# Aedelon/MASt3R-SLAM

Measured on AMD Instinct MI355X. Metric: keyframe-pairs/sec (512x512 two-view infer+match+GN), higher is better.
Workload: dtype fp16

## Files before the change

mast3r-slam_amd/csrc/gemm.hip:

```cpp
#include <atomic>
#include "gemm_common.h"
#include <cmath>
#include <stdlib.h>

using namespace m3gemm;

namespace {

constexpr int BM = 128, BN = 128;
constexpr int kThreads = 256;

#ifndef M3_GEMM64_STAGES
#define M3_GEMM64_STAGES 2
#endif
constexpr int k_gemm_stages(int T) { return T == 64 ? M3_GEMM64_STAGES : 2; }

template <int MODE , int EPI, int T, int DT, bool SLICED = false>
__global__ void __launch_bounds__(kThreads)
k_gemm(const GemmArgs gin) {
    constexpr int BM = T, BN = T;
    constexpr int NT = T / 32;
    constexpr int kStageBytes = (BM + BN) * BK * 2;
    constexpr int STAGES = k_gemm_stages(T);
    static_assert(4 * (NT == 4 ? 9216 : 4608) + BM * 8 + kRopeTableRows * 128 <= STAGES * kStageBytes, "row table + RoPE table behind the scratch");
// ... 330 lines not shown
    store_tile<EPI, DT>(g, f32x4{a.x, a.y, a.z, a.w}, m, n);
}

template <int MODE>
int run_split(const GemmArgs &a, int S, int epi, void *ws, hipStream_t st) {
    if (MODE == 1 && (epi == EPI_BF16 || epi == EPI_BF16_RELU || epi == EPI_BF16_ADD)) {
        const long tiles = (long)m3_cdiv(a.M, BM) * m3_cdiv(a.N, BN) * (a.groups > 1 ? a.groups : 1);
        static const bool sliced_ok = [] { const char *e = getenv("M3_CONV_SLICED"); return !(e && atoi(e) == 0); }();
        if (sliced_ok && tiles >= m3_device_cu_count()) {
            GemmArgs q = a;
            q.slices = S; q.splits = 1;
            return launch<MODE>(q, epi, st);
        }
    }
    GemmArgs p = a;
    p.C = ws; p.ldc = a.N; p.bias = nullptr; p.bias2 = nullptr; p.R = nullptr; p.splits = S;
    p.c_gstride = (long long)S * a.M * a.N;
    const int rc = launch<MODE>(p, EPI_F32, st);
    if (rc != M3_OK) return rc;
    const dim3 grid((unsigned)m3_cdiv((long)a.M * (a.N / 4), 256L), a.groups > 1 ? a.groups : 1);
#define M3_F(E) case E:                                                                                        \
        if (a.dt == DT_F16) hipLaunchKernelGGL((k_splitk_finish<E, DT_F16>), grid, dim3(256), 0, st, a, (const float *)ws, S); \
        else hipLaunchKernelGGL((k_splitk_finish<E, DT_BF16>), grid, dim3(256), 0, st, a, (const float *)ws, S);      \
        break
    switch (epi) {
        M3_F(EPI_BF16); M3_F(EPI_BF16_GELU); M3_F(EPI_F32); M3_F(EPI_F32_ACCUM); M3_F(EPI_BF16_RELU); M3_F(EPI_BF16_ADD);
        default: return M3_ERR_INVALID_ARG;
    }
#undef M3_F
    M3_CHECK_LAUNCH("m3_gemm/splitk_finish");
    return M3_OK;
}

}

int m3_launch_gemm256_dense(const GemmArgs &a, int epi, int bn, hipStream_t st);
int m3_launch_gemm256_conv(const GemmArgs &a, int epi, hipStream_t st);

static int launch_dense(const GemmArgs &a, int epi, hipStream_t st) {
    const int tile = pick_tile(a.M, a.N, a.groups > 1 ? 2 : 1);
    if (tile >= 192) return m3_launch_gemm256_dense(a, epi, tile, st);
    if (tile == 64) return launch<0, 64>(a, epi, st);
    return launch<0>(a, epi, st);
}

extern "C" {

int m3_gemm_set_tile(int tile) { return g_forced_tile.exchange(tile, std::memory_order_relaxed); }

int m3_gemm_pick_tile(int M, int N, int groups) {
    if (M <= 0 || N <= 0) return 0;
    return pick_tile(M, N, groups > 1 ? groups : 1);
}

static bool dt_ok(int dtype) { return dtype == DT_BF16 || dtype == DT_F16; }

static int ln_top_width(int C) {
    if (C % 192 == 0 && C / 192 <= 4) return 192;
    if (C % 256 == 0 && C / 256 <= 4) return 256;
    return 0;
}
static int ln_store_width(int M, int N, int groups) {
    const int tile = pick_tile(M, N, groups), top = ln_top_width(N);
    if (top == 0) return 0;
    if (tile == top) return top;
    if (top == 256 && tile == 128) return 128;
    return 64;
}
int m3_ln_slot_count(int M, int N, int groups) {
    if (M <= 0 || N <= 0) return 0;
    const int w = ln_store_width(M, N, groups > 1 ? 2 : 1);
    return w ? N / w : 0;
}

int m3_gemm_ex(const m3_gemm_desc *d, void *stream) {
    M3_REQUIRE(d && d->A && d->W && (d->C || d->c_lo) && d->M > 0 && d->N > 0 && d->K > 0);
    const int epi = d->epilogue, groups = d->groups > 1 ? 2 : 1;
    const bool rope = epi == EPI_BF16_ROPE;
    M3_REQUIRE(dt_ok(d->dtype) || (rope && d->dtype == 2));
    M3_REQUIRE(d->K % BK == 0 && d->N % 4 == 0 && d->ldc >= d->N && d->ldc % 4 == 0);
    M3_REQUIRE(!((epi == EPI_F32_ACCUM || epi == EPI_BF16_ADD) && !d->R));
    M3_REQUIRE(epi >= EPI_BF16 && epi <= EPI_BF16_ROPE);
    if (d->c_lo)
        M3_REQUIRE((epi == EPI_F32 || epi == EPI_F32_ACCUM) && d->dtype == DT_F16 && d->c16 && !d->C && d->N % 8 == 0 && d->ldc % 8 == 0 &&
                   d->M % 2 == 0 && (reinterpret_cast<size_t>(d->c_lo) & 15) == 0 && (reinterpret_cast<size_t>(d->c16) & 15) == 0 &&
                   (epi == EPI_F32 || (d->r_lo && (reinterpret_cast<size_t>(d->R) & 15) == 0 && (reinterpret_cast<size_t>(d->r_lo) & 15) == 0)));
    if (groups == 2) M3_REQUIRE(d->W1 && (d->bias == nullptr) == (d->bias1 == nullptr));
    if (rope)
        M3_REQUIRE(d->rope_pos && d->tokens_per_image > 0 && d->rope_base > 1.0f && d->N % 64 == 0 && d->rope_cols % 64 == 0 &&
                   d->rope_cols <= d->N && d->q_cols >= 0 && d->q_cols <= d->rope_cols && d->q_cols % 64 == 0);
    const bool f32out = epi == EPI_F32 || epi == EPI_F32_ACCUM;
    if (d->c16 || d->stats_out) {
        M3_REQUIRE(f32out && (d->N % 64 == 0 || !d->stats_out) && d->M % 2 == 0 && d->ldc % 8 == 0 && (reinterpret_cast<size_t>(d->C) & 15) == 0 &&
                   (!d->R || (reinterpret_cast<size_t>(d->R) & 15) == 0) &&
                   (!d->c16 || (reinterpret_cast<size_t>(d->c16) & 15) == 0) &&
                   (!d->stats_out || (reinterpret_cast<size_t>(d->stats_out) & 15) == 0));
        if (groups == 2) M3_REQUIRE(d->c_gstride % 8 == 0 && d->stats_gstride % 4 == 0);
        if (d->stats_out) M3_REQUIRE(d->stats_slots > 0 && d->stats_slots == m3_ln_slot_count(d->M, d->N, groups));
    }
    if (d->ln_stats) {
        const int top = ln_top_width(d->K);
        M3_REQUIRE(top != 0 && (d->ln_slots == d->K / 64 || (top == 256 && d->ln_slots == d->K / 128) || d->ln_slots == d->K / top));
        M3_REQUIRE(!f32out && epi != EPI_BF16_ADD && d->ln_colsum &&
                   d->ln_eps > 0.0f && d->M % 2 == 0 && (reinterpret_cast<size_t>(d->ln_stats) & 15) == 0 &&
                   (reinterpret_cast<size_t>(d->ln_colsum) & 15) == 0 && (reinterpret_cast<size_t>(d->C) & 15) == 0 &&
                   d->ldc % 8 == 0 && d->N % 8 == 0);
        if (groups == 2) M3_REQUIRE(d->ln_colsum1 && (reinterpret_cast<size_t>(d->ln_colsum1) & 15) == 0 && d->ln_gstride % 4 == 0);
    }
    GemmArgs a{};
    a.A = (const bf16_t *)d->A; a.W = (const bf16_t *)d->W; a.W2 = (const bf16_t *)d->W1; a.bias = d->bias; a.bias2 = d->bias1;
    a.C = d->C; a.R = d->R; a.M = d->M; a.N = d->N; a.K = d->K; a.ldc = d->ldc;
    a.dt = d->dtype == 2 ? DT_F16 : d->dtype; a.v_bf16 = d->dtype == 2;
    a.a_gstride = d->a_gstride; a.c_gstride = d->c_gstride; a.groups = groups == 2 ? 2 : 0;
    if (rope) {
        a.rope_pos = d->rope_pos; a.rope_log2_base = log2f(d->rope_base); a.tokens_per_image = d->tokens_per_image;
        a.rope_cols = d->rope_cols; a.q_cols = d->q_cols; a.q_scale = d->q_scale;
        a.rope_pmax = (d->rope_max_pos > 0 && d->rope_max_pos <= kRopeTableRows) ? d->rope_max_pos : 0;
    }
    a.C16 = d->c16; a.stats_out = d->stats_out; a.stats_gstride = d->stats_gstride;
    a.R_lo = d->r_lo; a.C_lo = d->c_lo;
    a.ln_stats = d->ln_stats; a.ln_colsum = d->ln_colsum; a.ln_colsum2 = d->ln_colsum1; a.ln_slots = d->ln_slots;
    a.ln_eps = d->ln_eps; a.ln_gstride = d->ln_gstride;
    if (d->ln_stats) {
        const int top = ln_top_width(d->K);
        a.ln_tops = d->K / top;
        a.ln_gsz = d->ln_slots / a.ln_tops;
    }
    a.stats_w = d->stats_out ? ln_store_width(d->M, d->N, groups) : 0;
    return launch_dense(a, epi, (hipStream_t)stream);
}

int64_t m3_conv3x3_splitk_bytes(int B, int H, int Wd, int Cin, int Cout, int stride) {
    if (B <= 0 || H <= 0 || Wd <= 0 || Cin <= 0 || Cout <= 0 || (stride != 1 && stride != 2)) return 0;
    const int OH = (H + 2 - 3) / stride + 1, OW = (Wd + 2 - 3) / stride + 1;
    const int S = pick_splits(OH * OW, Cout, 9 * Cin);
    return S > 1 ? (int64_t)S * B * OH * OW * Cout * 4 : 0;
}

int m3_conv3x3_grouped2_dt(const void *X, const void *W0, const void *W1, const float *bias0, const float *bias1,
                           void *Y, const void *R, const void *zero16, int B, int H, int Wd, int Cin, int Cout,
                           int stride, int epilogue, void *splitk_ws, int64_t splitk_ws_bytes, int dtype, void *stream) {
    const int relu_in = (epilogue & 0x100) ? 1 : 0;
    epilogue &= 0xff;
    M3_REQUIRE(X && W0 && Y && zero16 && B > 0 && H > 0 && Wd > 0 && Cin > 0 && Cout > 0 && dt_ok(dtype));
    M3_REQUIRE(Cin % BK == 0 && Cout % 4 == 0 && (stride == 1 || stride == 2) && epilogue != EPI_BF16_ROPE);
    M3_REQUIRE(!((epilogue == EPI_F32_ACCUM || epilogue == EPI_BF16_ADD) && !R));
    M3_REQUIRE(!W1 || (bias0 == nullptr) == (bias1 == nullptr));
    GemmArgs a{};
    a.relu_a = relu_in;
    a.A = (const bf16_t *)X; a.W = (const bf16_t *)W0; a.bias = bias0; a.C = Y; a.R = R;
    a.zero16 = (const bf16_t *)zero16;
    a.H = H; a.Wd = Wd; a.Cin = Cin; a.stride = stride;
    a.OH = (H + 2 - 3) / stride + 1; a.OW = (Wd + 2 - 3) / stride + 1;
    a.M = B * a.OH * a.OW; a.N = Cout; a.K = 9 * Cin; a.ldc = Cout; a.dt = dtype;
    if (W1) {
        a.W2 = (const bf16_t *)W1; a.bias2 = bias1;
        a.groups = 2; a.a_gstride = (long long)B * H * Wd * Cin; a.c_gstride = (long long)a.M * Cout;
    }
    const int S = pick_splits(a.OH * a.OW, Cout, a.K);
    if (S > 1) {
        M3_REQUIRE(splitk_ws && (reinterpret_cast<size_t>(splitk_ws) & 15) == 0 &&
                   splitk_ws_bytes >= (W1 ? 2 : 1) * (int64_t)S * a.M * a.N * 4);
        return run_split<1>(a, S, epilogue, splitk_ws, (hipStream_t)stream);
    }
    if (use_256(a.M, a.N, W1 ? 2 : 1)) return m3_launch_gemm256_conv(a, epilogue, (hipStream_t)stream);
    return launch<1>(a, epilogue, (hipStream_t)stream);
}

int m3_conv3x3_relu_head4_dt(const void *X, const void *W, const float *bias, const void *W4, const float *b4,
                             float *pts, float *conf, const void *zero16, int B, int H, int Wd, int Cin, int dtype,
                             void *stream) {
    M3_REQUIRE(X && W && W4 && b4 && pts && conf && zero16 && B > 0 && H > 0 && Wd > 0 && Cin > 0 && Cin % BK == 0);
    M3_REQUIRE(dt_ok(dtype));
    M3_REQUIRE((int64_t)B * H * Wd < (1ll << 31));
    GemmArgs a{};
    a.A = (const bf16_t *)X; a.W = (const bf16_t *)W; a.bias = bias; a.C = pts; a.C2 = conf;
    a.W2 = (const bf16_t *)W4; a.bias2 = b4;
    a.zero16 = (const bf16_t *)zero16;
    a.H = H; a.Wd = Wd; a.Cin = Cin; a.stride = 1; a.OH = H; a.OW = Wd;
// ... 6 lines not shown
```

mast3r-slam_amd/csrc/gemm256.hip:

```cpp
#include "gemm_common.h"

using namespace m3gemm;

namespace {

constexpr int BM = 256;
constexpr int kThreads = 512;

template <int MODE , int EPI, int BN, int DT>
__global__ void __launch_bounds__(kThreads, 2)
k_gemm256(const GemmArgs gin) {
    constexpr int WN = BN == 256 ? 4 : 2, WM = 8 / WN;
    constexpr int NI = BM / WM / 16, NJ = BN / WN / 16;
    constexpr int WISS = BN / 64;
    constexpr int kStageBytes = (BM + BN) * BK * 2;
    static_assert(8 * (64 * (32 * NJ + 16)) + kRopeTableRows * 128 <= 2 * kStageBytes, "RoPE table behind the epilogue scratch");
    const GemmArgs g = select_group<EPI>(gin, blockIdx.y);
    extern __shared__ __attribute__((aligned(16))) unsigned char lds[];
    const int tid = threadIdx.x, lane = tid & 63, wave = tid >> 6;
    const int group = wave >> 2;
    const int wr = wave / WN, wc = wave % WN;

    const int tiles_n = (g.N + BN - 1) / BN, tiles_m = (g.M + BM - 1) / BM;
    const int bid = xcd_remap(blockIdx.x, tiles_m * tiles_n);
    constexpr int GM = 8;
    const int band = bid / (GM * tiles_n), first_m = band * GM;
    const int gsz = tiles_m - first_m < GM ? tiles_m - first_m : GM;
    const int in_band = bid - band * GM * tiles_n;
    const int tm = first_m + in_band % gsz, tn = in_band / gsz;
    const int m0 = tm * BM, n0 = tn * BN;

    const int srow = tid >> 3, sch = (tid & 7) ^ ((srow >> 1) & 7);
    const bf16_t *a_src[4];
    const bf16_t *w_src[WISS];
    int a_oy[4], a_ox[4];
    const bf16_t *a_img[4];
#pragma unroll
    for (int i = 0; i < WISS; ++i) {
        int n = n0 + i * 64 + srow;
        n = n < g.N ? n : g.N - 1;
        w_src[i] = g.W + (size_t)n * g.K + sch * 8;
    }
#pragma unroll
    for (int i = 0; i < 4; ++i) {
        int m = m0 + i * 64 + srow;
        m = m < g.M ? m : g.M - 1;
        if (MODE == 0) {
            a_src[i] = g.A + (size_t)m * g.K + sch * 8;
        } else {
            const int pix = g.OH * g.OW;
            const int b = m / pix, rem = m - b * pix;
            a_oy[i] = (rem / g.OW) * g.stride - 1;
            a_ox[i] = (rem % g.OW) * g.stride - 1;
            a_img[i] = g.A + (size_t)b * g.H * g.Wd * g.Cin + sch * 8;
        }
    }
    const int nk = g.K / BK;

    auto stage_a = [&](int kt, int buf) {
        unsigned char *base = lds + buf * kStageBytes;
        int ky = 0, kx = 0, c0 = 0;
        if (MODE == 1) {
            const int q = kt / 9, tap = kt - q * 9;
            c0 = q * BK;
            ky = tap / 3; kx = tap - ky * 3;
        }
#pragma unroll
        for (int i = 0; i < 4; ++i) {
            const void *src;
            if (MODE == 0) {
                src = a_src[i] + (size_t)kt * BK;
            } else {
                const int iy = a_oy[i] + ky, ix = a_ox[i] + kx;
                const bool in = (iy >= 0) && (iy < g.H) && (ix >= 0) && (ix < g.Wd);
                src = in ? (const void *)(a_img[i] + ((size_t)iy * g.Wd + ix) * g.Cin + c0) : (const void *)g.zero16;
            }
            glds16(src, base + i * 8192 + wave * 1024);
        }
    };
    auto stage_w = [&](int kt, int buf) {
        unsigned char *base = lds + buf * kStageBytes;
        const size_t koff = MODE == 1 ? conv_k_offset(kt, g.Cin) : (size_t)kt * BK;
#pragma unroll
        for (int i = 0; i < WISS; ++i)
            glds16(w_src[i] + koff, base + BM * BK * 2 + i * 8192 + wave * 1024);
    };
    auto stage = [&](int kt, int buf) { stage_a(kt, buf); stage_w(kt, buf); };

    f32x4 acc[NI][NJ];
#pragma unroll
// ... 15 lines not shown
    }

    bf16x8 af[NI], wf[NJ];
    auto read_frags = [&](int buf, int ks) {
        const unsigned char *base = lds + buf * kStageBytes;
#pragma unroll
        for (int j = 0; j < NJ; ++j) wf[j] = *reinterpret_cast<const bf16x8 *>(base + (w_off[j] ^ (ks << 6)));
#pragma unroll
        for (int i = 0; i < NI; ++i) af[i] = *reinterpret_cast<const bf16x8 *>(base + (a_off[i] ^ (ks << 6)));
        if (MODE == 1 && g.relu_a) {
#pragma unroll
            for (int i = 0; i < NI; ++i) af[i] = relu_frag(af[i]);
        }
    };
    auto mfma_all = [&]() {
        __builtin_amdgcn_s_setprio(1);
#pragma unroll
        for (int i = 0; i < NI; ++i)
#pragma unroll
            for (int j = 0; j < NJ; ++j)
                acc[i][j] = mfma16<DT>(wf[j], af[i], acc[i][j]);
        __builtin_amdgcn_s_setprio(0);
    };
    auto phase_end = [&]() {
        __builtin_amdgcn_sched_barrier(0);
        __builtin_amdgcn_s_barrier();
        __builtin_amdgcn_sched_barrier(0);
    };
    auto phase_end_wait = [&]() {
        __builtin_amdgcn_sched_barrier(0);
        asm volatile("s_waitcnt vmcnt(0)" ::: "memory");
        __builtin_amdgcn_s_barrier();
        __builtin_amdgcn_sched_barrier(0);
    };

    if (MODE == 0 && g.ln_stats) {
        float2 *lnt = reinterpret_cast<float2 *>(lds + 2 * kStageBytes);
        const LnLoads L = ln_row_issue<BM>(g, m0, tid);
        stage(0, 0);
        ln_table_store<BM>(lnt, ln_row_finish<BM>(g, L, m0, tid), tid);
    } else {
        stage(0, 0);
    }
    float2 *lnt = (MODE == 0 && g.ln_stats) ? reinterpret_cast<float2 *>(lds + 2 * kStageBytes) : nullptr;
    phase_end_wait();

    if (group == 0) {
        for (int kt = 0; kt < nk; ++kt) {
            const int buf = kt & 1;
            read_frags(buf, 0);
            if (kt + 1 < nk) stage_a(kt + 1, buf ^ 1);
            asm volatile("s_waitcnt lgkmcnt(0)" ::: "memory");
            phase_end();
            mfma_all();
            phase_end();
            read_frags(buf, 1);
            if (kt + 1 < nk) stage_w(kt + 1, buf ^ 1);
            asm volatile("s_waitcnt lgkmcnt(0)" ::: "memory");
            phase_end();
            mfma_all();
            phase_end_wait();
        }
        phase_end();
    } else {
        for (int kt = 0; kt < nk; ++kt) {
            const int buf = kt & 1;
            if (kt > 0) mfma_all();
            phase_end();
            read_frags(buf, 0);
            if (kt + 1 < nk) stage_a(kt + 1, buf ^ 1);
            asm volatile("s_waitcnt lgkmcnt(0)" ::: "memory");
            phase_end();
            if (kt + 1 < nk) stage_w(kt + 1, buf ^ 1);
            mfma_all();
            phase_end();
            read_frags(buf, 1);
            asm volatile("s_waitcnt lgkmcnt(0)" ::: "memory");
            phase_end_wait();
        }
        mfma_all();
        phase_end();
    }

    const float *ropet = nullptr;
    if constexpr (EPI == EPI_BF16_ROPE && MODE == 0) {
        if (g.rope_pos && g.rope_pmax > 0) {
            float *tab = reinterpret_cast<float *>(lds + 8 * (64 * (32 * NJ + 16)));
            rope_table_build(g, tab, tid, kThreads);
            __syncthreads();
            ropet = tab;
        }
    }
    epilogue_rows<EPI, NI, NJ, DT>(g, acc, lds + wave * (64 * (32 * NJ + 16)), m0 + wr * (16 * NI), n0 + wc * (16 * NJ), lane, lnt,
                                   wr * (16 * NI), ropet);
    if constexpr (MODE == 0 && (EPI == EPI_F32 || EPI == EPI_F32_ACCUM)) {
        if (g.stats_out) {
            __syncthreads();
            stats_tile_finalize<BM, NI, NJ, WN>(g, lds, 64 * (32 * NJ + 16), stats_stage_offset<NJ>(), m0, n0, tid);
        }
    }
}

template <int MODE, int BN, int DT>
int launch256(const GemmArgs &a, int epi, hipStream_t st) {
    constexpr int kLdsBytes = 2 * (BM + BN) * BK * 2 + BM * 8;
    const int tiles = m3_cdiv(a.M, BM) * m3_cdiv(a.N, BN);
    dim3 grid(tiles, a.groups > 1 ? a.groups : 1), blk(kThreads);
#define M3_L(E)                                                                                              \
    case E: {                                                                                                \
        static M3AttrOnce once;                                                                              \
        int dev__;                                                                                           \
        if (m3_attr_need(once, &dev__)) {                                                                    \
            M3_CHECK_HIP(hipFuncSetAttribute(reinterpret_cast<const void *>(&k_gemm256<MODE, E, BN, DT>),        \
                                             hipFuncAttributeMaxDynamicSharedMemorySize, kLdsBytes),         \
                         "m3_gemm256/attr");                                                                 \
            m3_attr_done(once, dev__);                                                                       \
        }                                                                                                    \
        hipLaunchKernelGGL((k_gemm256<MODE, E, BN, DT>), grid, blk, kLdsBytes, st, a);                           \
    } break
    switch (epi) {
        M3_L(EPI_BF16); M3_L(EPI_BF16_GELU); M3_L(EPI_F32); M3_L(EPI_F32_ACCUM); M3_L(EPI_BF16_RELU); M3_L(EPI_BF16_ADD); M3_L(EPI_BF16_ROPE);
        default: return M3_ERR_INVALID_ARG;
    }
#undef M3_L
    M3_CHECK_LAUNCH("m3_gemm256");
    return M3_OK;
}

}

int m3_launch_gemm256_dense(const GemmArgs &a, int epi, int bn, hipStream_t st) {
    if (a.dt == DT_F16) return bn == 192 ? launch256<0, 192, DT_F16>(a, epi, st) : launch256<0, 256, DT_F16>(a, epi, st);
    return bn == 192 ? launch256<0, 192, DT_BF16>(a, epi, st) : launch256<0, 256, DT_BF16>(a, epi, st);
}
int m3_launch_gemm256_conv(const GemmArgs &a, int epi, hipStream_t st) {
    return a.dt == DT_F16 ? launch256<1, 256, DT_F16>(a, epi, st) : launch256<1, 256, DT_BF16>(a, epi, st);
}
```

mast3r-slam_amd/csrc/gemm_common.h:

```cpp
#pragma once
#include "common.h"
#include "../../include/m3slam_model.h"

namespace m3gemm {

typedef __attribute__((ext_vector_type(8))) short bf16x8;
typedef __attribute__((ext_vector_type(4))) float f32x4;
typedef unsigned short bf16_t;

constexpr int BK = 64;

__device__ __forceinline__ float bf2f(bf16_t v) { return __uint_as_float((unsigned)v << 16); }
__device__ __forceinline__ bf16_t f2bf(float f) {
    unsigned u = __float_as_uint(f);
    if ((u & 0x7fffffffu) > 0x7f800000u) return (bf16_t)((u >> 16) | 0x40);
    return (bf16_t)((u + 0x7fffu + ((u >> 16) & 1u)) >> 16);
}
typedef float f32x2 __attribute__((ext_vector_type(2)));
__device__ __forceinline__ f32x2 gelu_erf2(f32x2 x) {
    f32x2 z = x * 0.70710678118654752f;
    z.x = __builtin_amdgcn_fmed3f(z.x, -3.0f, 3.0f);
    z.y = __builtin_amdgcn_fmed3f(z.y, -3.0f, 3.0f);
    const f32x2 u = z * z;
    f32x2 p = (f32x2)(4.074053805e-08f);
// ... 256 lines not shown
__device__ __forceinline__ float2 ln_mean_rstd(float s, float q, int cols, float eps) {
    const float inv = 1.0f / (float)cols;
    const float mean = s * inv;
    const float var = fmaxf(__builtin_fmaf(-mean, mean, q * inv), 0.f);
    return make_float2(mean, rsqrtf(var + eps));
}
template <int ROWS>
__device__ __forceinline__ LnLoads ln_row_issue(const GemmArgs &g, int m0, int tid) {
    LnLoads L;
    const int pair = (tid < 2 * ROWS ? tid : 0) >> 2, q = tid & 3;
    const int node = q < g.ln_tops ? q : g.ln_tops - 1;
    int m = m0 + 2 * pair;
    m = m < g.M - 1 ? m : g.M - 2;
    const float4 *p = reinterpret_cast<const float4 *>(g.ln_stats + ((size_t)node * g.ln_gsz * g.M + m) * 2);
    const size_t slot_stride = (size_t)g.M / 2;
#pragma unroll
    for (int i = 0; i < 4; ++i) L.v[i] = p[(size_t)(i < g.ln_gsz ? i : g.ln_gsz - 1) * slot_stride];
    return L;
}
template <int ROWS>
__device__ __forceinline__ float4 ln_row_finish(const GemmArgs &g, const LnLoads &L, int m0, int tid) {
    const bool live = (tid & 3) < g.ln_tops;
    float4 u[4];
#pragma unroll
    for (int i = 0; i < 4; ++i) {
        const bool on = live && i < g.ln_gsz;
        u[i] = make_float4(on ? L.v[i].x : 0.f, on ? L.v[i].y : 0.f, on ? L.v[i].z : 0.f, on ? L.v[i].w : 0.f);
    }
    const float node[4] = {(u[0].x + u[1].x) + (u[2].x + u[3].x), (u[0].y + u[1].y) + (u[2].y + u[3].y),
                           (u[0].z + u[1].z) + (u[2].z + u[3].z), (u[0].w + u[1].w) + (u[2].w + u[3].w)};
    float t[4];
#pragma unroll
    for (int k = 0; k < 4; ++k) {
        const int b = __builtin_bit_cast(int, node[k]);
        const float t0 = __builtin_bit_cast(float, __builtin_amdgcn_update_dpp(0, b, 0x00, 0xF, 0xF, true));
        const float t1 = __builtin_bit_cast(float, __builtin_amdgcn_update_dpp(0, b, 0x55, 0xF, 0xF, true));
        const float t2 = __builtin_bit_cast(float, __builtin_amdgcn_update_dpp(0, b, 0xAA, 0xF, 0xF, true));
        const float t3 = __builtin_bit_cast(float, __builtin_amdgcn_update_dpp(0, b, 0xFF, 0xF, 0xF, true));
        t[k] = ((t0 + t1) + t2) + t3;
    }
    const float2 a = ln_mean_rstd(t[0], t[1], g.K, g.ln_eps), b2 = ln_mean_rstd(t[2], t[3], g.K, g.ln_eps);
    return make_float4(a.x, a.y, b2.x, b2.y);
}
template <int ROWS>
__device__ __forceinline__ float4 ln_row_stats(const GemmArgs &g, int m0, int tid) {
    return ln_row_finish<ROWS>(g, ln_row_issue<ROWS>(g, m0, tid), m0, tid);
}
template <int NJ> constexpr int stats_stage_offset() { return (16 * ((NJ == 4) ? 256 : NJ * 64 + 16) + 15) & ~15; }
template <int TROWS, int NI, int NJ, int WN>
__device__ __forceinline__ void stats_tile_finalize(const GemmArgs &g, const unsigned char *lds, int wave_stride, int wst_off,
                                                    int m0, int n0, int tid) {
    constexpr int WROWS = 16 * NI, LPW = NJ / 2, LEAVES = WN * LPW;
    if (tid >= TROWS) return;
    const int wr = tid / WROWS, rr = tid - wr * WROWS;
    const int lpu = g.stats_w >> 5;
    const int m = m0 + tid;
    for (int k = 0; k * lpu < LEAVES; ++k) {
        float s[8], q[8];
#pragma unroll
        for (int i = 0; i < 8; ++i) {
            const bool on = i < lpu;
            const int l = k * lpu + (on ? i : 0);
            const int wc = l / LPW, sl = l - wc * LPW;
            const float2 v = *reinterpret_cast<const float2 *>(lds + (wr * WN + wc) * wave_stride + wst_off + (sl * WROWS + rr) * 8);
            s[i] = on ? v.x : 0.f; q[i] = on ? v.y : 0.f;
        }
        const int n = n0 + k * g.stats_w;
        if (m < g.M && n < g.N)
            *reinterpret_cast<float2 *>(g.stats_out + ((size_t)(n / g.stats_w) * g.M + m) * 2) = make_float2(ln_tree8(s), ln_tree8(q));
    }
}
template <int ROWS>
__device__ __forceinline__ void ln_table_store(float2 *tab, const float4 &mr, int tid) {
    if (tid < 2 * ROWS && (tid & 3) == 0) {
        tab[2 * (tid >> 2)] = make_float2(mr.x, mr.y);
        tab[2 * (tid >> 2) + 1] = make_float2(mr.z, mr.w);
    }
}
template <int ROWS>
__device__ __forceinline__ void ln_row_table(const GemmArgs &g, float2 *tab, int m0, int tid) {
    ln_table_store<ROWS>(tab, ln_row_stats<ROWS>(g, m0, tid), tid);
}

template <int EPI, int NI, int NJ = 4, int DT = DT_BF16, int TPMAX = 4, bool RESID_AHEAD = true, bool ALIGNED = false>
__device__ __forceinline__ void epilogue_rows(const GemmArgs &g, f32x4 (&acc)[NI][NJ], unsigned char *wlds,
                                              int m_base, int n_base, int lane, const float2 *lnt = nullptr, int lrow = 0,
                                              const float *ropet = nullptr) {
    constexpr bool F32OUT = (EPI == EPI_F32 || EPI == EPI_F32_ACCUM);
    constexpr bool F32LDS = F32OUT || EPI == EPI_BF16_ADD;
    const int r = lane & 15, gq = lane >> 4;
    const bool aligned = ((reinterpret_cast<size_t>(g.C) & 15) == 0) && (g.ldc % (F32OUT ? 4 : 8) == 0) &&
                         (F32OUT || g.N % 8 == 0) &&
                         (!(EPI == EPI_F32_ACCUM || EPI == EPI_BF16_ADD) || (reinterpret_cast<size_t>(g.R) & 15) == 0);
    if (!ALIGNED && !aligned) {
#pragma unroll
        for (int i = 0; i < NI; ++i) {
            if (EPI == EPI_BF16_ROPE) rope_strip<NJ>(g, acc[i], m_base + i * 16 + r, n_base, lane);
#pragma unroll
            for (int j = 0; j < NJ; ++j) store_tile<EPI, DT>(g, acc[i][j], m_base + i * 16 + r, n_base + j * 16 + gq * 4);
        }
        return;
    }
    float4 bj[NJ];
    if (g.bias) {
#pragma unroll
        for (int j = 0; j < NJ; ++j) {
            const int n = n_base + j * 16 + gq * 4;
            bj[j] = *reinterpret_cast<const float4 *>(g.bias + (n < g.N ? n : g.N - 4));
        }
#pragma unroll
        for (int j = 0; j < NJ; ++j)
            if (n_base + j * 16 + gq * 4 >= g.N) bj[j] = make_float4(0.f, 0.f, 0.f, 0.f);
    } else {
#pragma unroll
        for (int j = 0; j < NJ; ++j) bj[j] = make_float4(0.f, 0.f, 0.f, 0.f);
    }
    if (F32LDS) {
        constexpr bool SWZ32 = F32OUT && (NJ == 4);
        constexpr int RS = SWZ32 ? 256 : NJ * 64 + 16;
        constexpr bool RESID = (EPI == EPI_F32_ACCUM || EPI == EPI_BF16_ADD);
        constexpr int PT = 1;
        constexpr int PR = 16 * PT;
        constexpr int CPR = F32OUT ? NJ * 4 : NJ * 2;
        constexpr int NIT = PR * CPR / 64;
        static_assert(!F32OUT || ((PR * RS + 15) & ~15) == stats_stage_offset<NJ>(), "stats_tile_finalize reads the staging where the epilogue wrote it");
        float2 *wst = reinterpret_cast<float2 *>(wlds + ((PR * RS + 15) & ~15));
        uint4 q[RESID_AHEAD ? 2 : 1][RESID ? NIT : 1];
        auto load_resid = [&](int pass, uint4 (&dst)[RESID ? NIT : 1]) {
            if constexpr (RESID) {
                size_t off[NIT];
#pragma unroll
                for (int it = 0; it < NIT; ++it) {
                    const int c = it * 64 + lane, rl = c / CPR, ch = c - rl * CPR;
                    int m = m_base + pass * PR + rl, n = n_base + ch * (F32OUT ? 4 : 8);
                    m = m < g.M ? m : g.M - 1;
                    n = n < g.N ? n : 0;
                    off[it] = (size_t)m * g.ldc + n;
                }
                if (F32OUT && g.C_lo) {
#pragma unroll
                    for (int it = 0; it < NIT; ++it) {
                        const uint2 hi = *reinterpret_cast<const uint2 *>(reinterpret_cast<const bf16_t *>(g.R) + off[it]);
                        const uint2 lo = *reinterpret_cast<const uint2 *>(reinterpret_cast<const bf16_t *>(g.R_lo) + off[it]);
                        dst[it] = uint4{hi.x, hi.y, lo.x, lo.y};
                    }
                } else {
#pragma unroll
                    for (int it = 0; it < NIT; ++it)
                        dst[it] = F32OUT ? *reinterpret_cast<const uint4 *>(reinterpret_cast<const float *>(g.R) + off[it])
                                         : *reinterpret_cast<const uint4 *>(reinterpret_cast<const bf16_t *>(g.R) + off[it]);
                }
            }
        };
        if (RESID_AHEAD) load_resid(0, q[0]);
#pragma unroll
        for (int pass = 0; pass < NI / PT; ++pass) {
            if (RESID_AHEAD) { if (pass + 1 < NI / PT) load_resid(pass + 1, q[(pass + 1) & (RESID_AHEAD ? 1 : 0)]); }
            else load_resid(pass, q[0]);
#pragma unroll
            for (int ii = 0; ii < PT; ++ii)
#pragma unroll
                for (int j = 0; j < NJ; ++j) {
                    const f32x4 v = acc[pass * PT + ii][j];
                    *reinterpret_cast<float4 *>(wlds + (ii * 16 + r) * RS + ((SWZ32 ? ((j * 4 + gq) ^ (r & 7)) : (j * 4 + gq)) << 4)) =
                        make_float4(v[0] + bj[j].x, v[1] + bj[j].y, v[2] + bj[j].z, v[3] + bj[j].w);
                }
            asm volatile("s_waitcnt lgkmcnt(0)" ::: "memory");
            if (F32OUT) {
#pragma unroll
                for (int it = 0; it < NIT; ++it) {
                    const int c = it * 64 + lane, rl = c / CPR, ch = c - rl * CPR;
                    float4 v = *reinterpret_cast<const float4 *>(wlds + rl * RS + ((SWZ32 ? (ch ^ (rl & 7)) : ch) << 4));
                    const int m = m_base + pass * PR + rl, n = n_base + ch * 4;
                    if (EPI == EPI_F32_ACCUM) {
                        const uint4 u = q[RESID_AHEAD ? (pass & 1) : 0][it];
                        if (g.C_lo) {
                            v.x += lo16<DT>(u.x) + lo16<DT>(u.z); v.y += hi16<DT>(u.x) + hi16<DT>(u.z);
                            v.z += lo16<DT>(u.y) + lo16<DT>(u.w); v.w += hi16<DT>(u.y) + hi16<DT>(u.w);
                        } else {
                            v.x += __uint_as_float(u.x); v.y += __uint_as_float(u.y); v.z += __uint_as_float(u.z); v.w += __uint_as_float(u.w);
                        }
                    }
                    if (g.C_lo) {
                        const unsigned h0 = pack16<DT>(v.x, v.y), h1 = pack16<DT>(v.z, v.w);
                        const unsigned l0 = pack16<DT>(v.x - lo16<DT>(h0), v.y - hi16<DT>(h0));
                        const unsigned l1 = pack16<DT>(v.z - lo16<DT>(h1), v.w - hi16<DT>(h1));
                        const unsigned g0 = dpp_xor1(h0), g1 = dpp_xor1(h1), k0 = dpp_xor1(l0), k1 = dpp_xor1(l1);
                        if (!(lane & 1) && m < g.M && n < g.N) {
                            *reinterpret_cast<uint4 *>(reinterpret_cast<bf16_t *>(g.C16) + (size_t)m * g.ldc + n) = uint4{h0, h1, g0, g1};
                            *reinterpret_cast<uint4 *>(reinterpret_cast<bf16_t *>(g.C_lo) + (size_t)m * g.ldc + n) = uint4{l0, l1, k0, k1};
                        }
                    } else {
                    if (m < g.M && n < g.N)
                        *reinterpret_cast<float4 *>(reinterpret_cast<float *>(g.C) + (size_t)m * g.ldc + n) = v;
                    if (g.C16) {
                        const unsigned p0 = pack16<DT>(v.x, v.y), p1 = pack16<DT>(v.z, v.w);
                        const unsigned q0 = dpp_xor1(p0), q1 = dpp_xor1(p1);
                        if (!(lane & 1) && m < g.M && n < g.N)
                            *reinterpret_cast<uint4 *>(reinterpret_cast<bf16_t *>(g.C16) + (size_t)m * g.ldc + n) = uint4{p0, p1, q0, q1};
                    }
                    }
                    if (g.stats_out) {
                        const bool live = m < g.M && n < g.N;
                        const float s1 = dpp_sum8(live ? (v.x + v.y) + (v.z + v.w) : 0.f);
                        const float s2 = dpp_sum8(live ? (v.x * v.x + v.y * v.y) + (v.z * v.z + v.w * v.w) : 0.f);
                        if ((ch & 7) == 0)
                            wst[(ch >> 3) * (16 * NI) + pass * PR + rl] = make_float2(s1, s2);
                    }
                }
            } else {
#pragma unroll
                for (int it = 0; it < NIT; ++it) {
                    const int c = it * 64 + lane, rl = c / CPR, ch = c - rl * CPR;
                    const float4 a = *reinterpret_cast<const float4 *>(wlds + rl * RS + ch * 32);
                    const float4 b = *reinterpret_cast<const float4 *>(wlds + rl * RS + ch * 32 + 16);
                    const int m = m_base + pass * PR + rl, n = n_base + ch * 8;
                    const uint4 u = q[RESID_AHEAD ? (pass & 1) : 0][it];
                    uint4 o;
                    o.x = pack16<DT>(a.x + lo16<DT>(u.x), a.y + hi16<DT>(u.x));
                    o.y = pack16<DT>(a.z + lo16<DT>(u.y), a.w + hi16<DT>(u.y));
                    o.z = pack16<DT>(b.x + lo16<DT>(u.z), b.y + hi16<DT>(u.z));
                    o.w = pack16<DT>(b.z + lo16<DT>(u.w), b.w + hi16<DT>(u.w));
                    if (m < g.M && n < g.N)
                        *reinterpret_cast<uint4 *>(reinterpret_cast<bf16_t *>(g.C) + (size_t)m * g.ldc + n) = o;
                }
            }
            asm volatile("" ::: "memory");
        }
    } else {
        constexpr bool SWZ = (NJ == 4);
        constexpr int RS = SWZ ? 128 : NJ * 32 + 16;
        constexpr int TP = NI < TPMAX ? NI : TPMAX;
        constexpr int PR = 16 * TP, CPR = NJ * 2;
        RopeFreq fr{};
        if constexpr (EPI == EPI_BF16_ROPE) { if (g.rope_pos && !ropet) fr = rope_freqs(g, lane); }
        if (lnt) {
            float4 csj[NJ];
#pragma unroll
            for (int j = 0; j < NJ; ++j) {
                const int n = n_base + j * 16 + gq * 4;
                csj[j] = *reinterpret_cast<const float4 *>(g.ln_colsum + (n < g.N ? n : g.N - 4));
            }
#pragma unroll
            for (int i = 0; i < NI; ++i) {
                const float2 mr = lnt[lrow + i * 16 + r];
#pragma unroll
                for (int j = 0; j < NJ; ++j) {
                    f32x4 &v = acc[i][j];
                    v[0] = mr.y * (v[0] - mr.x * csj[j].x); v[1] = mr.y * (v[1] - mr.x * csj[j].y);
                    v[2] = mr.y * (v[2] - mr.x * csj[j].z); v[3] = mr.y * (v[3] - mr.x * csj[j].w);
                }
            }
        }
#pragma unroll
        for (int pass = 0; pass < NI / TP; ++pass) {
            RopeCoef cf[EPI == EPI_BF16_ROPE ? TP : 1][NJ / 2];
            if constexpr (EPI == EPI_BF16_ROPE) {
                int2 pyx[TP];
#pragma unroll
                for (int ii = 0; ii < TP; ++ii) pyx[ii] = int2{0, 0};
                if (g.rope_pos) {
#pragma unroll
                    for (int ii = 0; ii < TP; ++ii) pyx[ii] = rope_pos_of(g, m_base + (pass * TP + ii) * 16 + r);
                }
#pragma unroll
                for (int ii = 0; ii < TP; ++ii) rope_load<NJ>(g, cf[ii], n_base, lane, fr, pyx[ii], ropet);
            }
#pragma unroll
            for (int ii = 0; ii < TP; ++ii) {
                const int i = pass * TP + ii;
                if constexpr (EPI == EPI_BF16_ROPE) rope_apply<NJ>(g, acc[i], cf[ii], bj, n_base);
#pragma unroll
                for (int j = 0; j < NJ; ++j) {
                    f32x4 v = acc[i][j];
                    if constexpr (EPI != EPI_BF16_ROPE) { v[0] += bj[j].x; v[1] += bj[j].y; v[2] += bj[j].z; v[3] += bj[j].w; }
                    if (EPI == EPI_BF16_GELU) {
                        const f32x2 lo = gelu_erf2(f32x2{v[0], v[1]}), hi = gelu_erf2(f32x2{v[2], v[3]});
                        v[0] = lo.x; v[1] = lo.y; v[2] = hi.x; v[3] = hi.y;
                    }
                    if (EPI == EPI_BF16_RELU) {
#pragma unroll
                        for (int e = 0; e < 4; ++e) v[e] = v[e] > 0.f ? v[e] : 0.f;
                    }
                    uint2 pk;
                    if (EPI == EPI_BF16_ROPE && DT == DT_F16 && g.v_bf16 && n_base + (j >> 1) * 32 >= g.rope_cols) {
                        pk.x = pack16<DT_BF16>(v[0], v[1]); pk.y = pack16<DT_BF16>(v[2], v[3]);
                    } else {
                        pk.x = pack16<DT>(v[0], v[1]); pk.y = pack16<DT>(v[2], v[3]);
                    }
                    if constexpr (SWZ)
                        *reinterpret_cast<uint2 *>(wlds + (ii * 16 + r) * RS + (((j * 2 + (gq >> 1)) ^ ((r >> 1) & 7)) << 4) + (((gq ^ r) & 1) << 3)) = pk;
                    else
                        *reinterpret_cast<uint2 *>(wlds + (ii * 16 + r) * RS + (j * 16 + gq * 4) * 2) = pk;
                }
            }
            asm volatile("s_waitcnt lgkmcnt(0)" ::: "memory");
#pragma unroll
            for (int it = 0; it < PR * CPR / 64; ++it) {
                const int c = it * 64 + lane, rl = c / CPR, ch = c - rl * CPR;
                uint4 v = *reinterpret_cast<const uint4 *>(wlds + rl * RS + ((SWZ ? (ch ^ ((rl >> 1) & 7)) : ch) << 4));
                if (SWZ && (rl & 1)) v = uint4{v.z, v.w, v.x, v.y};
                const int m = m_base + pass * PR + rl, n = n_base + ch * 8;
                if (m < g.M && n < g.N)
                    *reinterpret_cast<uint4 *>(reinterpret_cast<bf16_t *>(g.C) + (size_t)m * g.ldc + n) = v;
            }
            asm volatile("" ::: "memory");
        }
    }
}

__device__ __forceinline__ size_t conv_k_offset(int kt, int Cin) {
// ... 11 lines not shown
```

Measured before the change: 294.4.

## Split hi/lo residual traffic across lane pairs in the fp32-accum GEMM epilogue

Reworks the fp32-output GEMM epilogue for the split hi/lo fp16 residual stream. Odd lanes load and store the low half while even lanes handle the high half with full 16-byte accesses, and DPP lane swaps exchange the data, replacing paired 8-byte loads and half-idle stores. The bias add moves into the accumulators before staging, and the prefetch depth plus stats presence become compile-time variants. Host alignment checks are relaxed to allow a narrower fallback path. Ablation macros (default off) are added for probing, and the extra template variants increase code size and register pressure.

```diff
diff --git a/mast3r-slam_amd/csrc/gemm.hip b/mast3r-slam_amd/csrc/gemm.hip
--- a/mast3r-slam_amd/csrc/gemm.hip
+++ b/mast3r-slam_amd/csrc/gemm.hip
@@ -436,19 +436,20 @@
     M3_REQUIRE(!((epi == EPI_F32_ACCUM || epi == EPI_BF16_ADD) && !d->R));
     M3_REQUIRE(epi >= EPI_BF16 && epi <= EPI_BF16_ROPE);
     if (d->c_lo)
-        M3_REQUIRE((epi == EPI_F32 || epi == EPI_F32_ACCUM) && d->dtype == DT_F16 && d->c16 && !d->C && d->N % 8 == 0 && d->ldc % 8 == 0 &&
-                   d->M % 2 == 0 && (reinterpret_cast<size_t>(d->c_lo) & 15) == 0 && (reinterpret_cast<size_t>(d->c16) & 15) == 0 &&
-                   (epi == EPI_F32 || (d->r_lo && (reinterpret_cast<size_t>(d->R) & 15) == 0 && (reinterpret_cast<size_t>(d->r_lo) & 15) == 0)));
+        M3_REQUIRE((epi == EPI_F32 || epi == EPI_F32_ACCUM) && d->dtype == DT_F16 && d->c16 && !d->C &&
+                   d->M % 2 == 0 && (reinterpret_cast<size_t>(d->c_lo) & 7) == 0 && (reinterpret_cast<size_t>(d->c16) & 7) == 0 &&
+                   (epi == EPI_F32 || (d->r_lo && (reinterpret_cast<size_t>(d->R) & 7) == 0 && (reinterpret_cast<size_t>(d->r_lo) & 7) == 0)));
     if (groups == 2) M3_REQUIRE(d->W1 && (d->bias == nullptr) == (d->bias1 == nullptr));
     if (rope)
         M3_REQUIRE(d->rope_pos && d->tokens_per_image > 0 && d->rope_base > 1.0f && d->N % 64 == 0 && d->rope_cols % 64 == 0 &&
                    d->rope_cols <= d->N && d->q_cols >= 0 && d->q_cols <= d->rope_cols && d->q_cols % 64 == 0);
     const bool f32out = epi == EPI_F32 || epi == EPI_F32_ACCUM;
     if (d->c16 || d->stats_out) {
-        M3_REQUIRE(f32out && (d->N % 64 == 0 || !d->stats_out) && d->M % 2 == 0 && d->ldc % 8 == 0 && (reinterpret_cast<size_t>(d->C) & 15) == 0 &&
-                   (!d->R || (reinterpret_cast<size_t>(d->R) & 15) == 0) &&
-                   (!d->c16 || (reinterpret_cast<size_t>(d->c16) & 15) == 0) &&
+        M3_REQUIRE(f32out && (d->N % 64 == 0 || !d->stats_out) && d->M % 2 == 0 &&
                    (!d->stats_out || (reinterpret_cast<size_t>(d->stats_out) & 15) == 0));
+        if (!d->c_lo)
+            M3_REQUIRE(d->ldc % 8 == 0 && (reinterpret_cast<size_t>(d->C) & 15) == 0 && (!d->R || (reinterpret_cast<size_t>(d->R) & 15) == 0) &&
+                       (!d->c16 || (reinterpret_cast<size_t>(d->c16) & 15) == 0));
         if (groups == 2) M3_REQUIRE(d->c_gstride % 8 == 0 && d->stats_gstride % 4 == 0);
         if (d->stats_out) M3_REQUIRE(d->stats_slots > 0 && d->stats_slots == m3_ln_slot_count(d->M, d->N, groups));
     }
diff --git a/mast3r-slam_amd/csrc/gemm256.hip b/mast3r-slam_amd/csrc/gemm256.hip
--- a/mast3r-slam_amd/csrc/gemm256.hip
+++ b/mast3r-slam_amd/csrc/gemm256.hip
@@ -6,6 +6,12 @@
 
 constexpr int BM = 256;
 constexpr int kThreads = 512;
+#ifndef M3_RESID_AHEAD_256
+#define M3_RESID_AHEAD_256 1
+#endif
+#ifndef M3_RESID_AHEAD_192
+#define M3_RESID_AHEAD_192 1
+#endif
 
 template <int MODE , int EPI, int BN, int DT>
 __global__ void __launch_bounds__(kThreads, 2)
@@ -187,6 +193,7 @@
         phase_end();
     }
 
+    if constexpr (EPI == EPI_F32_ACCUM && (M3_RESID_ABL & 16)) { abl_keep(acc); return; }
     const float *ropet = nullptr;
     if constexpr (EPI == EPI_BF16_ROPE && MODE == 0) {
         if (g.rope_pos && g.rope_pmax > 0) {
@@ -196,10 +203,12 @@
             ropet = tab;
         }
     }
-    epilogue_rows<EPI, NI, NJ, DT>(g, acc, lds + wave * (64 * (32 * NJ + 16)), m0 + wr * (16 * NI), n0 + wc * (16 * NJ), lane, lnt,
+    int lane_e = lane;
+    asm volatile("" : "+v"(lane_e));
+    epilogue_rows<EPI, NI, NJ, DT, 4, EPI == EPI_F32_ACCUM ? (BN == 256 ? M3_RESID_AHEAD_256 : M3_RESID_AHEAD_192) : 1>(g, acc, lds + wave * (64 * (32 * NJ + 16)), m0 + wr * (16 * NI), n0 + wc * (16 * NJ), lane_e, lnt,
                                    wr * (16 * NI), ropet);
     if constexpr (MODE == 0 && (EPI == EPI_F32 || EPI == EPI_F32_ACCUM)) {
-        if (g.stats_out) {
+        if (g.stats_out && !(EPI == EPI_F32_ACCUM && (M3_RESID_ABL & 4))) {
             __syncthreads();
             stats_tile_finalize<BM, NI, NJ, WN>(g, lds, 64 * (32 * NJ + 16), stats_stage_offset<NJ>(), m0, n0, tid);
         }
diff --git a/mast3r-slam_amd/csrc/gemm_common.h b/mast3r-slam_amd/csrc/gemm_common.h
--- a/mast3r-slam_amd/csrc/gemm_common.h
+++ b/mast3r-slam_amd/csrc/gemm_common.h
@@ -362,16 +362,29 @@
     ln_table_store<ROWS>(tab, ln_row_stats<ROWS>(g, m0, tid), tid);
 }
 
-template <int EPI, int NI, int NJ = 4, int DT = DT_BF16, int TPMAX = 4, bool RESID_AHEAD = true, bool ALIGNED = false>
+#ifndef M3_RESID_ABL
+#define M3_RESID_ABL 0
+#endif
+template <int V> struct StreamForm { static constexpr int value = V; };
+template <int NI, int NJ> __device__ __forceinline__ void abl_keep(f32x4 (&acc)[NI][NJ]) {
+#pragma unroll
+    for (int i = 0; i < NI; ++i)
+#pragma unroll
+        for (int j = 0; j < NJ; ++j) asm volatile("" ::"v"(acc[i][j]));
+}
+
+template <int EPI, int NI, int NJ = 4, int DT = DT_BF16, int TPMAX = 4, int AHEAD = 1, bool ALIGNED = false>
 __device__ __forceinline__ void epilogue_rows(const GemmArgs &g, f32x4 (&acc)[NI][NJ], unsigned char *wlds,
                                               int m_base, int n_base, int lane, const float2 *lnt = nullptr, int lrow = 0,
                                               const float *ropet = nullptr) {
     constexpr bool F32OUT = (EPI == EPI_F32 || EPI == EPI_F32_ACCUM);
     constexpr bool F32LDS = F32OUT || EPI == EPI_BF16_ADD;
+    constexpr int ABL = EPI == EPI_F32_ACCUM ? M3_RESID_ABL : 0;
     const int r = lane & 15, gq = lane >> 4;
-    const bool aligned = ((reinterpret_cast<size_t>(g.C) & 15) == 0) && (g.ldc % (F32OUT ? 4 : 8) == 0) &&
-                         (F32OUT || g.N % 8 == 0) &&
-                         (!(EPI == EPI_F32_ACCUM || EPI == EPI_BF16_ADD) || (reinterpret_cast<size_t>(g.R) & 15) == 0);
+    const bool aligned = (F32OUT && g.C_lo) ||
+                         (((reinterpret_cast<size_t>(g.C) & 15) == 0) && (g.ldc % (F32OUT ? 4 : 8) == 0) &&
+                          (F32OUT || g.N % 8 == 0) &&
+                          (!(EPI == EPI_F32_ACCUM || EPI == EPI_BF16_ADD) || (reinterpret_cast<size_t>(g.R) & 15) == 0));
     if (!ALIGNED && !aligned) {
 #pragma unroll
         for (int i = 0; i < NI; ++i) {
@@ -405,23 +418,50 @@
         constexpr int NIT = PR * CPR / 64;
         static_assert(!F32OUT || ((PR * RS + 15) & ~15) == stats_stage_offset<NJ>(), "stats_tile_finalize reads the staging where the epilogue wrote it");
         float2 *wst = reinterpret_cast<float2 *>(wlds + ((PR * RS + 15) & ~15));
-        uint4 q[RESID_AHEAD ? 2 : 1][RESID ? NIT : 1];
+        if constexpr (!(ABL & 8)) {
+#pragma unroll
+            for (int i = 0; i < NI; ++i)
+#pragma unroll
+                for (int j = 0; j < NJ; ++j) acc[i][j] += f32x4{bj[j].x, bj[j].y, bj[j].z, bj[j].w};
+        }
+        constexpr int NPASS = NI / PT, QN = AHEAD + 1;
+        bool wide = false;
+        if constexpr (F32OUT) {
+            wide = g.C_lo && g.N % 8 == 0 && g.ldc % 8 == 0 &&
+                   ((reinterpret_cast<size_t>(g.C16) | reinterpret_cast<size_t>(g.C_lo)) & 15) == 0 &&
+                   (EPI != EPI_F32_ACCUM || ((reinterpret_cast<size_t>(g.R) | reinterpret_cast<size_t>(g.R_lo)) & 15) == 0);
+        }
+        const bool odd = lane & 1;
+        const bf16_t *const r_hi = reinterpret_cast<const bf16_t *>(g.R), *const r_lo = reinterpret_cast<const bf16_t *>(g.R_lo);
+        bf16_t *const c_hi = reinterpret_cast<bf16_t *>(g.C16), *const c_lo = reinterpret_cast<bf16_t *>(g.C_lo);
+        const bf16_t *const r_mine = odd ? r_lo : r_hi;
+        bf16_t *const c_mine = odd ? c_lo : c_hi;
+        auto run = [&](auto form, auto with_stats) __attribute__((always_inline)) {
+        constexpr int FORM = decltype(form)::value, STATS = decltype(with_stats)::value;
+        const bool stats = F32OUT && !(ABL & 4) && (STATS < 0 ? g.stats_out != nullptr : STATS != 0);
+        uint4 q[QN][RESID ? NIT : 1];
         auto load_resid = [&](int pass, uint4 (&dst)[RESID ? NIT : 1]) {
-            if constexpr (RESID) {
+            if constexpr (RESID && (ABL & 1)) {
+#pragma unroll
+                for (int it = 0; it < NIT; ++it) dst[it] = uint4{0x3c003c00u, 0x3c003c00u, 0u, 0u};
+            } else if constexpr (RESID) {
                 size_t off[NIT];
 #pragma unroll
                 for (int it = 0; it < NIT; ++it) {
                     const int c = it * 64 + lane, rl = c / CPR, ch = c - rl * CPR;
-                    int m = m_base + pass * PR + rl, n = n_base + ch * (F32OUT ? 4 : 8);
+                    int m = m_base + pass * PR + rl, n = n_base + (FORM == 2 ? (ch & ~1) : ch) * (F32OUT ? 4 : 8);
                     m = m < g.M ? m : g.M - 1;
                     n = n < g.N ? n : 0;
                     off[it] = (size_t)m * g.ldc + n;
                 }
-                if (F32OUT && g.C_lo) {
+                if constexpr (FORM == 2) {
+#pragma unroll
+                    for (int it = 0; it < NIT; ++it) dst[it] = *reinterpret_cast<const uint4 *>(r_mine + off[it]);
+                } else if constexpr (FORM == 1) {
 #pragma unroll
                     for (int it = 0; it < NIT; ++it) {
-                        const uint2 hi = *reinterpret_cast<const uint2 *>(reinterpret_cast<const bf16_t *>(g.R) + off[it]);
-                        const uint2 lo = *reinterpret_cast<const uint2 *>(reinterpret_cast<const bf16_t *>(g.R_lo) + off[it]);
+                        const uint2 hi = *reinterpret_cast<const uint2 *>(r_hi + off[it]);
+                        const uint2 lo = *reinterpret_cast<const uint2 *>(r_lo + off[it]);
                         dst[it] = uint4{hi.x, hi.y, lo.x, lo.y};
                     }
                 } else {
@@ -432,55 +472,66 @@
                 }
             }
         };
-        if (RESID_AHEAD) load_resid(0, q[0]);
-#pragma unroll
-        for (int pass = 0; pass < NI / PT; ++pass) {
-            if (RESID_AHEAD) { if (pass + 1 < NI / PT) load_resid(pass + 1, q[(pass + 1) & (RESID_AHEAD ? 1 : 0)]); }
+#pragma unroll
+        for (int p = 0; p < AHEAD && p < NPASS; ++p) load_resid(p, q[p % QN]);
+#pragma unroll
+        for (int pass = 0; pass < NPASS; ++pass) {
+            if (AHEAD > 0) { if (pass + AHEAD < NPASS) load_resid(pass + AHEAD, q[(pass + AHEAD) % QN]); }
             else load_resid(pass, q[0]);
-#pragma unroll
-            for (int ii = 0; ii < PT; ++ii)
+            if constexpr ((ABL & 8) != 0) abl_keep(acc);
+#pragma unroll
+            for (int ii = 0; ii < ((ABL & 8) ? 0 : PT); ++ii)
 #pragma unroll
                 for (int j = 0; j < NJ; ++j) {
                     const f32x4 v = acc[pass * PT + ii][j];
                     *reinterpret_cast<float4 *>(wlds + (ii * 16 + r) * RS + ((SWZ32 ? ((j * 4 + gq) ^ (r & 7)) : (j * 4 + gq)) << 4)) =
-                        make_float4(v[0] + bj[j].x, v[1] + bj[j].y, v[2] + bj[j].z, v[3] + bj[j].w);
+                        make_float4(v[0], v[1], v[2], v[3]);
                 }
             asm volatile("s_waitcnt lgkmcnt(0)" ::: "memory");
             if (F32OUT) {
 #pragma unroll
                 for (int it = 0; it < NIT; ++it) {
                     const int c = it * 64 + lane, rl = c / CPR, ch = c - rl * CPR;
-                    float4 v = *reinterpret_cast<const float4 *>(wlds + rl * RS + ((SWZ32 ? (ch ^ (rl & 7)) : ch) << 4));
+                    float4 v = (ABL & 8) ? bj[it % NJ] : *reinterpret_cast<const float4 *>(wlds + rl * RS + ((SWZ32 ? (ch ^ (rl & 7)) : ch) << 4));
                     const int m = m_base + pass * PR + rl, n = n_base + ch * 4;
                     if (EPI == EPI_F32_ACCUM) {
-                        const uint4 u = q[RESID_AHEAD ? (pass & 1) : 0][it];
-                        if (g.C_lo) {
+                        uint4 u = q[pass % QN][it];
+                        if constexpr (FORM == 2) {
+                            const unsigned r0 = dpp_xor1(odd ? u.x : u.z), r1 = dpp_xor1(odd ? u.y : u.w);
+                            u = odd ? uint4{r0, r1, u.z, u.w} : uint4{u.x, u.y, r0, r1};
+                        }
+                        if constexpr (FORM != 0) {
                             v.x += lo16<DT>(u.x) + lo16<DT>(u.z); v.y += hi16<DT>(u.x) + hi16<DT>(u.z);
                             v.z += lo16<DT>(u.y) + lo16<DT>(u.w); v.w += hi16<DT>(u.y) + hi16<DT>(u.w);
                         } else {
                             v.x += __uint_as_float(u.x); v.y += __uint_as_float(u.y); v.z += __uint_as_float(u.z); v.w += __uint_as_float(u.w);
                         }
                     }
-                    if (g.C_lo) {
+                    if constexpr ((ABL & 2) != 0) {
+                    } else if constexpr (FORM != 0) {
                         const unsigned h0 = pack16<DT>(v.x, v.y), h1 = pack16<DT>(v.z, v.w);
                         const unsigned l0 = pack16<DT>(v.x - lo16<DT>(h0), v.y - hi16<DT>(h0));
                         const unsigned l1 = pack16<DT>(v.z - lo16<DT>(h1), v.w - hi16<DT>(h1));
-                        const unsigned g0 = dpp_xor1(h0), g1 = dpp_xor1(h1), k0 = dpp_xor1(l0), k1 = dpp_xor1(l1);
-                        if (!(lane & 1) && m < g.M && n < g.N) {
-                            *reinterpret_cast<uint4 *>(reinterpret_cast<bf16_t *>(g.C16) + (size_t)m * g.ldc + n) = uint4{h0, h1, g0, g1};
-                            *reinterpret_cast<uint4 *>(reinterpret_cast<bf16_t *>(g.C_lo) + (size_t)m * g.ldc + n) = uint4{l0, l1, k0, k1};
+                        if constexpr (FORM == 2) {
+                            const unsigned r0 = dpp_xor1(odd ? h0 : l0), r1 = dpp_xor1(odd ? h1 : l1);
+                            const uint4 o = odd ? uint4{r0, r1, l0, l1} : uint4{h0, h1, r0, r1};
+                            const int np = n_base + (ch & ~1) * 4;
+                            if (m < g.M && np < g.N) *reinterpret_cast<uint4 *>(c_mine + (size_t)m * g.ldc + np) = o;
+                        } else if (m < g.M && n < g.N) {
+                            *reinterpret_cast<uint2 *>(c_hi + (size_t)m * g.ldc + n) = uint2{h0, h1};
+                            *reinterpret_cast<uint2 *>(c_lo + (size_t)m * g.ldc + n) = uint2{l0, l1};
                         }
                     } else {
-                    if (m < g.M && n < g.N)
-                        *reinterpret_cast<float4 *>(reinterpret_cast<float *>(g.C) + (size_t)m * g.ldc + n) = v;
-                    if (g.C16) {
-                        const unsigned p0 = pack16<DT>(v.x, v.y), p1 = pack16<DT>(v.z, v.w);
-                        const unsigned q0 = dpp_xor1(p0), q1 = dpp_xor1(p1);
-                        if (!(lane & 1) && m < g.M && n < g.N)
-                            *reinterpret_cast<uint4 *>(reinterpret_cast<bf16_t *>(g.C16) + (size_t)m * g.ldc + n) = uint4{p0, p1, q0, q1};
+                        if (m < g.M && n < g.N)
+                            *reinterpret_cast<float4 *>(reinterpret_cast<float *>(g.C) + (size_t)m * g.ldc + n) = v;
+                        if (g.C16) {
+                            const unsigned p0 = pack16<DT>(v.x, v.y), p1 = pack16<DT>(v.z, v.w);
+                            const unsigned q0 = dpp_xor1(p0), q1 = dpp_xor1(p1);
+                            if (!odd && m < g.M && n < g.N)
+                                *reinterpret_cast<uint4 *>(c_hi + (size_t)m * g.ldc + n) = uint4{p0, p1, q0, q1};
+                        }
                     }
-                    }
-                    if (g.stats_out) {
+                    if (stats) {
                         const bool live = m < g.M && n < g.N;
                         const float s1 = dpp_sum8(live ? (v.x + v.y) + (v.z + v.w) : 0.f);
                         const float s2 = dpp_sum8(live ? (v.x * v.x + v.y * v.y) + (v.z * v.z + v.w * v.w) : 0.f);
@@ -495,7 +546,7 @@
                     const float4 a = *reinterpret_cast<const float4 *>(wlds + rl * RS + ch * 32);
                     const float4 b = *reinterpret_cast<const float4 *>(wlds + rl * RS + ch * 32 + 16);
                     const int m = m_base + pass * PR + rl, n = n_base + ch * 8;
-                    const uint4 u = q[RESID_AHEAD ? (pass & 1) : 0][it];
+                    const uint4 u = q[pass % QN][it];
                     uint4 o;
                     o.x = pack16<DT>(a.x + lo16<DT>(u.x), a.y + hi16<DT>(u.x));
                     o.y = pack16<DT>(a.z + lo16<DT>(u.y), a.w + hi16<DT>(u.y));
@@ -507,6 +558,11 @@
             }
             asm volatile("" ::: "memory");
         }
+        };
+        if (wide && g.stats_out) run(StreamForm<F32OUT ? 2 : 0>{}, StreamForm<1>{});
+        else if (wide) run(StreamForm<F32OUT ? 2 : 0>{}, StreamForm<0>{});
+        else if (F32OUT && g.C_lo) run(StreamForm<F32OUT ? 1 : 0>{}, StreamForm<-1>{});
+        else run(StreamForm<0>{}, StreamForm<-1>{});
     } else {
         constexpr bool SWZ = (NJ == 4);
         constexpr int RS = SWZ ? 128 : NJ * 32 + 16;
```

Result: no change. 292.7 (-0.6%).
